# Chlumsky/msdfgen

Hardware: AMD Instinct MI355X
Metric: MSDF glyphs/sec (64x64, fp32) (higher is better)
Workload: dtype f64

## Files before the change

### msdfgen_amd/csrc/msdf_capi.hip

```cpp

#include <hip/hip_runtime.h>

#include <algorithm>
#include <atomic>
#include <chrono>
#include <condition_variable>
#include <cmath>
#include <cstdarg>
#include <cstdio>
#include <cstdlib>
#include <cstring>
#include <deque>
#include <functional>
#include <memory>
#include <mutex>
#include <string>
#include <thread>
#include <vector>

#include <sched.h>

#include "msdf_classplan.hpp"
#include "msdf_hostplan.hpp"
#include "msdf_kernels.hpp"
// ... 645 lines not shown
            rc = fail(MSDFHIP_ERR_HIP, "joining the glyph-class streams failed: %s", hipGetErrorString(joinError));
    }
    if (rc == MSDFHIP_OK && plan.unculled)
        rc = unculled(b, dGlyphs, w, h, dst, toScratch, stream, plan.unculledMapped ? b->work.bucket.ptr+plan.unculledOffset : NULL, plan.unculledCount, call.boxDims);
    return rc;
}

size_t candidateRecords(int nGlyphs, size_t texelsPerGlyph) { return ecHeaderRecords(nGlyphs)+(size_t) nGlyphs*ecSegment(texelsPerGlyph); }
size_t offsetRecords(int nGlyphs) { return (ecOffsetInts(nGlyphs)*sizeof(int)+sizeof(EcCandidate)-1)/sizeof(EcCandidate); }
size_t deferredRecords(int nGlyphs, size_t texelsPerGlyph, int nEdges) {
    return candidateRecords(nGlyphs, texelsPerGlyph)+offsetRecords(nGlyphs)+((size_t) (nEdges > 0 ? nEdges : 1)*2*sizeof(int)+sizeof(EcCandidate)-1)/sizeof(EcCandidate);
}

int ensureDeferred(const MsdfHipBatch *b, size_t cap, EcCandidate **out) {
    std::lock_guard<std::mutex> lock(b->work.mutex);
    HIPCHK(b->work.deferred.ensure(cap));
    HIPCHK(b->work.ecParams.ensure(b->work.glyphCapacity(b->nGlyphs)));
    *out = b->work.deferred.ptr;
    return MSDFHIP_OK;
}

template <int N, bool OVERLAP>
unsigned queryResidentBlocks(int device, size_t lds) {
    enum { LDS_STEP = 2048, LDS_STEPS = 81 };
    static std::atomic<int> cache[LDS_STEPS];
    const size_t step = (lds+LDS_STEP-1)/LDS_STEP;
    return step < LDS_STEPS ? (unsigned) residentBlocks(cache[step], device, reinterpret_cast<const void *>(k_ec_query<N, OVERLAP>), WAVE, step*LDS_STEP) : 0u;
}

template <int N, bool OVERLAP, bool GRES>
int launchEc(const MsdfHipBatch *b, const MsdfHipGlyph *dGlyphs, int w, int h, const float *src, float *out, uint8_t *stencil,
             const MsdfHipConfig &cfg, hipStream_t stream, GenerateCall &call, bool paramsOnly, const EcPlan &p) {
    const int tilesX = (w+TILE-1)/TILE, tiles = tilesOf(w, h);
    const unsigned blocks = (unsigned) b->nGlyphs*(unsigned) tiles;
    if (p.tooManyTexels)
        return fail(MSDFHIP_ERR_INVALID, "batch of %zu texels exceeds the 32-bit texel index of the error-correction pass; split the batch", p.allTexels);
    double *gres = NULL;
    int rc;
    if (GRES) {
        rc = ensureGres(b, (size_t) p.slowGrid*p.resBytes, &gres);
        if (rc != MSDFHIP_OK)
            return rc;
    }
    const size_t gresStride = p.resBytes/sizeof(double);
    const int32_t *dDims = call.boxDims;
    auto slowKernel = k_ec_slow<N, OVERLAP, GRES>;
    auto fastKernel = p.lazyProtect ? k_ec_fast<N, true> : k_ec_fast<N, false>;
    if (call.ecShapeRows) {
        if constexpr (!OVERLAP && !GRES) {
            if (dDims || p.lazyProtect)
                return fail(MSDFHIP_ERR_INVALID, "a correction along the shape's rows takes neither boxes of their own sizes nor the distance check");
            slowKernel = k_ec_slow<N, false, false, true>;
            fastKernel = k_ec_fast<N, false, true>;
        } else
            return fail(MSDFHIP_ERR_INVALID, "a correction along the shape's rows runs without overlap support");
    }
    const auto slowTwin = ecSlowSizedKernel(N, OVERLAP, GRES);
    const auto fastTwin = ecFastSizedKernel(N, p.lazyProtect);
    const auto queryTwin = ecQuerySizedKernel(N, OVERLAP);
    const BatchView v = viewOf(b);
    rc = setLdsTwinned(slowKernel, slowTwin, dDims, p.slowLds);
    if (rc != MSDFHIP_OK)
        return rc;
    ScopedTimer timer(stream, 1, !paramsOnly);
    if (p.route == EC_ROUTE_STAGE_SNAPSHOT || p.route == EC_ROUTE_SLOW_ALL) {
        if (paramsOnly)
            return MSDFHIP_OK;
        launchTwinned(slowKernel, slowTwin, dDims, dim3(p.route == EC_ROUTE_SLOW_ALL ? p.slowGrid : p.snapshotBlocks), p.slowLds, stream, v, dGlyphs, w, h, src, out,
                      stencil, cfg, NULL, 0u, 0, gres, gresStride);
        HIPCHK(hipGetLastError());
        if (p.route == EC_ROUTE_SLOW_ALL)
            countRoute(MSDFHIP_ROUTE_EC_SLOW_ALL);
        return MSDFHIP_OK;
    }
    const unsigned seg = ecSegment((size_t) w*h);
    EcCandidate *deferred = NULL;
    rc = ensureDeferred(b, deferredRecords(b->nGlyphs, (size_t) w*h, b->nEdges), &deferred);
    if (rc != MSDFHIP_OK)
        return rc;
    if (p.route == EC_ROUTE_TOO_COMPLEX)
        return fail(MSDFHIP_ERR_TOO_COMPLEX, "a glyph has %d contours / %d edges: the error-correction pass needs %zu B of LDS per wavefront, device limit is %d B",
                    b->maxContours, b->maxEdges, p.fastLds > p.queryLds ? p.fastLds : p.queryLds, gLdsLimit.load());
    rc = setLdsTwinned(k_ec_query<N, OVERLAP>, queryTwin, dDims, p.queryLds);
    if (rc != MSDFHIP_OK)
        return rc;
    rc = setLdsTwinned(fastKernel, fastTwin, dDims, p.fastLds);
    if (rc != MSDFHIP_OK)
        return rc;
    int *offsets = reinterpret_cast<int *>(deferred+candidateRecords(b->nGlyphs, (size_t) w*h));
    int *corners = reinterpret_cast<int *>(deferred+candidateRecords(b->nGlyphs, (size_t) w*h)+offsetRecords(b->nGlyphs));
    const unsigned queryBlocks = p.residentQueryBlocks(p.staticDeal ? queryResidentBlocks<N, OVERLAP>(b->device, p.queryLds) : 0u);
    const EcQueryPolicy policy = { p.lpcMaxContours, p.lpcEdgeCost, p.lpcMaxEdges, p.lpcMinCount, p.wideMaxEdges, p.wideLoad, p.wideMeanCount, p.gridSteps };
    if (!call.ecParamsQueued)
        hipLaunchKernelGGL(k_ec_params, dim3((unsigned) b->nGlyphs), dim3(WAVE), 0, stream, b->work.ecParams.ptr, viewOf(b), dGlyphs, cfg,
                           reinterpret_cast<unsigned *>(deferred), corners, offsets+ecSizesAt(b->nGlyphs));
    const int *ecOrder = NULL;
    rc = ensureEcOrder(b, &ecOrder, stream);
    if (rc != MSDFHIP_OK)
        return rc;
    if (paramsOnly) {
        HIPCHK(hipGetLastError());
        call.ecParamsQueued = true;
        return MSDFHIP_OK;
    }
    launchTwinned(fastKernel, fastTwin, dDims, dim3(blocks), p.fastLds, stream, v, dGlyphs, w, h, tilesX, tiles, src, out, stencil, cfg, b->work.ecParams.ptr, deferred,
                  seg, b->maxEdges, corners);
    hipLaunchKernelGGL(k_ec_scan, dim3(1), dim3(1024), 0, stream, b->nGlyphs, reinterpret_cast<const unsigned *>(deferred), seg, offsets, policy, ecOrder);
    launchTwinned(k_ec_query<N, OVERLAP>, queryTwin, dDims, dim3(queryBlocks), p.queryLds, stream, v.nGlyphs, v.glyphContourOffsets, v.contourOffsets, v.recs, v.windings,
                  dGlyphs, w, h, src, out, stencil, cfg, b->work.ecParams.ptr, deferred, seg, offsets, offsets+2*(size_t) b->nGlyphs+2, p.queryBatch, p.slotCap,
                  p.slotOffset, policy, call.overflowOut, ecOrder, p.queryFlags);
    if (call.overflowOut)
        call.overflowMirrored = true;
    else
        launchTwinned(slowKernel, slowTwin, dDims, dim3(p.slowGrid), p.slowLds, stream, v, dGlyphs, w, h, src, out, stencil, cfg, deferred, seg, 1, gres, gresStride);
    HIPCHK(hipGetLastError());
    countRoute(ecOrder ? MSDFHIP_ROUTE_EC_QUERY_HEAVIEST : MSDFHIP_ROUTE_EC_QUERY_BATCH);
    if (p.wideSlots)
        countRoute(MSDFHIP_ROUTE_EC_WIDE_SLOTS);
    return MSDFHIP_OK;
}

template <int N>
int dispatchEc(const MsdfHipBatch *b, const MsdfHipGlyph *dGlyphs, int w, int h, const float *src, float *out, uint8_t *stencil,
               const MsdfHipConfig &cfg, hipStream_t stream, GenerateCall &call, bool paramsOnly) {
    const EcPlan p = planCorrection(planEnv(b->device), countsOf(b), w, h, N, cfg.overlap_support != 0, cfg.ec_mode, cfg.ec_distance_check, cfg.ec_stage_limit,
                                    ecFastLdsBytes(b->maxEdges, N));
    if (!cfg.overlap_support)
        return launchEc<N, false, false>(b, dGlyphs, w, h, src, out, stencil, cfg, stream, call, paramsOnly, p);
    return p.gres ? launchEc<N, true, true>(b, dGlyphs, w, h, src, out, stencil, cfg, stream, call, paramsOnly, p)
                  : launchEc<N, true, false>(b, dGlyphs, w, h, src, out, stencil, cfg, stream, call, paramsOnly, p);
}

int checkConfig(const MsdfHipConfig *cfg) {
    if (!cfg)
        return fail(MSDFHIP_ERR_INVALID, "cfg is NULL");
    if (cfg->ec_mode < 0 || cfg->ec_mode > 3 || cfg->ec_distance_check < 0 || cfg->ec_distance_check > 2 || cfg->ec_stage_limit < 0 || cfg->ec_stage_limit > 4)
        return fail(MSDFHIP_ERR_INVALID, "bad error-correction config (mode %d, distance check %d, stage limit %d)", cfg->ec_mode, cfg->ec_distance_check, cfg->ec_stage_limit);
    return MSDFHIP_OK;
}

int ensureScratch(const MsdfHipBatch *b, size_t floats, float **out) {
    std::lock_guard<std::mutex> lock(b->work.mutex);
    HIPCHK(b->work.scratch.ensure(floats));
    *out = b->work.scratch.ptr;
    return MSDFHIP_OK;
}

int runCorrection(const MsdfHipBatch *b, int channels, int w, int h, const MsdfHipGlyph *dGlyphs, const float *src, float *out, uint8_t *stencil,
                  const MsdfHipConfig &cfg, hipStream_t stream, GenerateCall &call, bool paramsOnly) {
    int rc = MSDFHIP_OK;
    forOneOf<3, 4>(channels, [&](auto n) { rc = dispatchEc<decltype(n)::value>(b, dGlyphs, w, h, src, out, stencil, cfg, stream, call, paramsOnly); });
    return rc;
}

int prepareAhead(const MsdfHipBatch *b, int mode, int w, int h, const MsdfHipGlyph *dGlyphs, const MsdfHipConfig *cfg, hipStream_t stream, GenerateCall &call) {
    if (b->nGlyphs == 0 || w == 0 || h == 0)
        return MSDFHIP_OK;
    const int nch = channelsOf(mode);
    int rc = MSDFHIP_OK;
// ... 3105 lines not shown
```

### msdfgen_amd/csrc/msdf_ec_fast.hpp

```cpp
#pragma once

#include "msdf_ec.hpp"

namespace msdfhip {

enum { EC_DEFER = 0x80 };

enum { EC_V_ERROR = 1,
       EC_V_CHECK = 2,
       EC_V_COND = 4,
       EC_V_HELD = 8 };
enum { EC_ORDER_EAGER = 0, EC_ORDER_LAZY = 1, EC_ORDER_LAZY_HELD = 2 };

MSDF_HD bool ecHasBasePass(const EcParams &p) { return p.distanceCheck == EC_DO_NOT_CHECK || (p.distanceCheck == EC_CHECK_AT_EDGE && p.mode != EC_MODE_EDGE_ONLY); }
MSDF_HD bool ecHasShapePass(const EcParams &p) { return p.distanceCheck == EC_ALWAYS_CHECK || p.distanceCheck == EC_CHECK_AT_EDGE; }
MSDF_HD bool ecLazyProtect(const EcParams &p) { return p.mode == EC_MODE_EDGE_PRIORITY && p.distanceCheck == EC_CHECK_AT_EDGE; }

struct FastCtx {
    double span;
    bool p1;
    bool pShape;
    bool basePass, shapePass;
    int order;
};
// ... 138 lines not shown
            break;
        const double t = i ? d.r1 : d.r0;
        const float xm = interpolatedMedianQuad<HWMED>(a, l, q, t);
        int rangeFlags = diagonalUnitFlags<HWMED>(cx, am, dm, a, l, q, t, 0, false, xm);
        if (d.ne > 0)
            rangeFlags |= diagonalUnitFlags<HWMED>(cx, am, dm, a, l, q, t, d.ex0, true, xm);
        if (d.ne > 1)
            rangeFlags |= diagonalUnitFlags<HWMED>(cx, am, dm, a, l, q, t, d.ex1, true, xm);
        if (diagonalRootVerdict(cx, rangeFlags, t, verdict, sink))
            return verdict;
    }
    return verdict;
}

struct Neighbourhood {
    float v[3][3][3];
    float dev[3][3];
    unsigned cls[3][3];
    unsigned valid;
};

template <bool HWMED = false>
MSDF_HD float ecTexelDeviation(const float *t) { return fabsf(medianOf<HWMED>(t[0], t[1], t[2])-.5f); }

enum { EC_CLS_INSIDE = 0x8000 };
MSDF_HD unsigned ecTexelClassWord(const float *t) {
    unsigned w = EC_CLS_INSIDE;
    MSDF_UNROLL
    for (int j = 0; j < 3; ++j) {
        const float d = t[j == 2 ? 0 : j+1]-t[j];
        w |= (d > 0 ? 1u<<j : 0u)|(d < 0 ? 8u<<j : 0u)|(d == 0 ? 64u<<j : 0u);
    }
    return w;
}

MSDF_HD unsigned ecValidFromWords(const Neighbourhood &nb) {
    unsigned valid = 0;
    MSDF_UNROLL
    for (int m = 0; m < 9; ++m)
        valid |= (nb.cls[m/3][m%3]&EC_CLS_INSIDE) ? 1u<<m : 0u;
    return valid;
}

MSDF_HD void loadNeighbourhood(Neighbourhood &nb, const SdfView &sdf, int x, int yn) {
    MSDF_UNROLL
    for (int dy = -1; dy <= 1; ++dy) {
        MSDF_UNROLL
        for (int dx = -1; dx <= 1; ++dx) {
            const int nx = x+dx, ny = yn+dy;
            const bool in = nx >= 0 && ny >= 0 && nx < sdf.w && ny < sdf.h;
            const float *t = sdf.native(in ? nx : x, in ? ny : yn);
            nb.v[dy+1][dx+1][0] = t[0], nb.v[dy+1][dx+1][1] = t[1], nb.v[dy+1][dx+1][2] = t[2];
            nb.dev[dy+1][dx+1] = ecTexelDeviation(t);
            nb.cls[dy+1][dx+1] = in ? ecTexelClassWord(t) : 0u;
        }
    }
    nb.valid = ecValidFromWords(nb);
}

enum { EC_PROTECT_TESTS = 8, EC_PROTECT_MASK = 0x1ef };
MSDF_HD unsigned texelProtectMask(const Neighbourhood &nb, const EcParams &p) {
    const float sdev = nb.dev[1][1];
    unsigned mask = 0;
    MSDF_UNROLL
    for (int dy = -1; dy <= 1; ++dy) {
        MSDF_UNROLL
// ... 235 lines not shown
```

### msdfgen_amd/csrc/msdf_kernels.hpp

```cpp
#pragma once

#include <hip/hip_runtime.h>
#include "msdf_device.hpp"
#include "msdf_prep.hpp"
#include "msdf_ec.hpp"
#include "msdf_ec_fast.hpp"
#include "msdf_cull.hpp"
#include "msdf_scanline.hpp"
#include "msdf_render.hpp"
#include "msdf_qualityplan.hpp"
#include "msdf_shapeprep.hpp"
#include "msdf_frame.hpp"
#include "msdf_legacy.hpp"
#include "../../include/msdfgen_hip.h"

namespace msdfhip {

#ifndef MSDF_DISTANCE_WAVES_PER_SIMD
#define MSDF_DISTANCE_WAVES_PER_SIMD 4
#endif
constexpr int TILE = 8;
constexpr int WAVE = 64;
constexpr int REC_DOUBLES = sizeof(EdgeRec)/sizeof(double);

// ... 974 lines not shown

template <class T, T V>
struct EcConstant {
    static constexpr T value = V;
};

__device__ __forceinline__ int waveInclusiveSum(int v) {
    v += __builtin_amdgcn_update_dpp(0, v, 0x111, 0xf, 0xf, false);
    v += __builtin_amdgcn_update_dpp(0, v, 0x112, 0xf, 0xf, false);
    v += __builtin_amdgcn_update_dpp(0, v, 0x114, 0xf, 0xf, false);
    v += __builtin_amdgcn_update_dpp(0, v, 0x118, 0xf, 0xf, false);
    v += __builtin_amdgcn_update_dpp(0, v, 0x142, 0xa, 0xf, false);
    v += __builtin_amdgcn_update_dpp(0, v, 0x143, 0xc, 0xf, false);
    return v;
}
struct EcWaveReserve {
    int *count;
    __device__ void operator()(int nFirst, int nOthers, int &atFirst, int &atOthers) {
        const int n = nFirst|nOthers<<16;
        const int through = waveInclusiveSum(n);
        const int total = __builtin_amdgcn_readlane(through, WAVE-1), before = through-n;
        *count = (total&0xffff)+(total>>16);
        atFirst = before&0xffff, atOthers = (total&0xffff)+(before>>16);
    }
};
template <unsigned VALID, int TESTS, unsigned FIRST>
__device__ __forceinline__ void ecAppendWave(unsigned short *queue, int *count, unsigned mask, int lane) {
    if (__ballot(mask != 0) == 0)
        return;
    EcWaveReserve reserve = { count };
    ecAppendItems<VALID, TESTS, FIRST>(queue, mask, lane, reserve);
}

template <int N, int ORDER = -1, bool SIZED = false, bool SHAPE_ROWS = false>
__device__ __forceinline__ void ecFastBody(const BatchView &batch, const MsdfHipGlyph *glyphs, int width, int height, int tilesX, int tilesPerGlyph,
          const float *src, float *out, uint8_t *stencilOut, const MsdfHipConfig &cfg, const EcGlyphParams *glyphParams, EcCandidate *cands, unsigned seg,
          int maxEdges, const int *corners, const unsigned blockId, int *smemFast, const int sinkSlots = 0, const int sinkSlot = 0, const int32_t *__restrict__ dims = NULL) {
    const GlyphWork wk = decodeItem(blockId, batch.nGlyphs, tilesPerGlyph);
    if (!wk.valid)
        return;
    const int boxW = SIZED ? MSDF_UNIFORM(dims[2*wk.g]) : width, boxH = SIZED ? MSDF_UNIFORM(dims[2*wk.g+1]) : height;
    if (SIZED && ((wk.tile%tilesX)*TILE >= boxW || (wk.tile/tilesX)*TILE >= boxH))
        return;
    float *halo = reinterpret_cast<float *>(smemFast);
    int *verdictLds = reinterpret_cast<int *>(halo+EC_HALO*EC_HALO*N);
    int *itemCount = verdictLds+WAVE;
    unsigned short *queue = reinterpret_cast<unsigned short *>(itemCount+4);
    unsigned short *protectQueue = queue+EC_QUEUE_CAP;
    struct TexelClass {
        float dev;
        unsigned cls;
    };
    TexelClass *classLds = reinterpret_cast<TexelClass *>(queue+EC_QUEUE_CAP)-EC_HALO*EC_HALO;
    static_assert((EC_QUEUE_CAP*sizeof(unsigned short))%sizeof(TexelClass) == 0 && EC_QUEUE_CAP*sizeof(unsigned short) >= EC_HALO*EC_HALO*sizeof(TexelClass)
                  && 2*WAVE >= EC_HALO*EC_HALO && WAVE%EC_HALO == 4 && WAVE/EC_HALO == 6, "classLds overlays the queue's tail; the halo is staged in two rounds");
    const int lane = threadIdx.x;
    const MsdfHipGlyph gd = glyphs[wk.g];
    EcParams p;
    p.t = loadXform(gd);
    p.minDeviationRatio = cfg.min_deviation_ratio;
    p.minImproveRatio = cfg.min_improve_ratio;
    constexpr bool FOLD = ORDER == 1 && !SIZED;
    p.mode = FOLD ? (int) EC_MODE_EDGE_PRIORITY : cfg.ec_mode, p.distanceCheck = FOLD ? (int) EC_CHECK_AT_EDGE : cfg.ec_distance_check;
    p.overlap = cfg.overlap_support, p.stageLimit = 0;
    const EcGlyphParams gp = glyphParams[wk.g];
    p.hSpan = gp.hSpan, p.vSpan = gp.vSpan, p.dSpan = gp.dSpan, p.texelX = gp.texelX, p.texelY = gp.texelY;
    p.radiusH = gp.radiusH, p.radiusV = gp.radiusV, p.radiusD = gp.radiusD;
    const int tx = wk.tile%tilesX, ty = wk.tile/tilesX;

    const bool lazy = ORDER < 0 ? ecLazyProtect(p) : ORDER != 0;
    bool cornerTexel = false;
    if (p.mode == EC_MODE_EDGE_PRIORITY && !lazy)
        cornerTexel = ecTileCornerTexel(corners+2*(size_t) gp.cornerBegin, gp.nCorners, tx, ty, boxH, gd.flip, lane);

    const ptrdiff_t rowStep = (ptrdiff_t) boxW*N;
    const ptrdiff_t origin = SIZED ? ((ptrdiff_t) wk.g*width*height+(ptrdiff_t) (ty*TILE-1)*boxW+tx*TILE-1)*N : (((ptrdiff_t) wk.g*height+ty*TILE-1)*width+tx*TILE-1)*N;
    const int hr0 = lane/EC_HALO, hc0 = lane-hr0*EC_HALO;
    const ptrdiff_t laneStep0 = hr0*rowStep+hc0*N;
    constexpr bool VOTE = ORDER >= 0 && !SIZED && !SHAPE_ROWS;
    constexpr bool INDEXED = VOTE;
    constexpr float EC_MED3_BOUND = 0x1p100f;
    bool objection = false;
    MSDF_UNROLL
    for (int round = 0; round < 2; ++round) {
        const int idx = lane+round*WAVE;
        const bool wrap = round && hc0+WAVE%EC_HALO >= EC_HALO;
        const int hc = hc0+round*(WAVE%EC_HALO)-(wrap ? EC_HALO : 0), hr = hr0+round*(WAVE/EC_HALO)+(wrap ? 1 : 0);
        const ptrdiff_t laneStep = laneStep0+round*((WAVE/EC_HALO)*rowStep+(WAVE%EC_HALO)*N)+(wrap ? rowStep-EC_HALO*N : 0);
        if (idx < EC_HALO*EC_HALO) {
            const int hx = tx*TILE+hc-1, hy = ty*TILE+hr-1;
            unsigned cls = 0;
            if (hx >= 0 && hy >= 0 && hx < boxW && hy < boxH) {
                const float *t = src+(origin+laneStep);
                float tv[N];
                for (int ch = 0; ch < N; ++ch)
                    tv[ch] = t[ch], halo[idx*N+ch] = tv[ch];
                if (VOTE)
                    objection = objection || !(fabsf(tv[0]) < EC_MED3_BOUND && fabsf(tv[1]) < EC_MED3_BOUND && fabsf(tv[2]) < EC_MED3_BOUND);
                classLds[idx].dev = ecTexelDeviation(tv);
                cls = ecTexelClassWord(tv);
            }
            classLds[idx].cls = cls;
        }
    }
    if (lane < 2)
        itemCount[lane] = 0;
    waveSync();

    const int lx = lane&(TILE-1), ly = lane>>3;
    const int x = tx*TILE+lx, yn = ty*TILE+ly;
    const bool inside = x < boxW && yn < boxH;
    int st = 0;
    const bool classify = inside;
    Neighbourhood nb;
    const int centre = (ly+1)*EC_HALO+lx+1;
    MSDF_UNROLL
    for (int dy = -1; dy <= 1; ++dy) {
        MSDF_UNROLL
        for (int dx = -1; dx <= 1; ++dx) {
            const TexelClass tc = classLds[centre+dy*EC_HALO+dx];
            nb.dev[dy+1][dx+1] = tc.dev, nb.cls[dy+1][dx+1] = tc.cls;
        }
    }
    waveSync();
    unsigned findMask = 0, protectMask = 0;
    const bool hwMedian = VOTE && __ballot(objection) == 0;
    if (classify) {
        MSDF_UNROLL
        for (int dy = -1; dy <= 1; ++dy) {
            MSDF_UNROLL
            for (int dx = -1; dx <= 1; ++dx) {
                const float *t = halo+(centre+dy*EC_HALO+dx)*N;
                nb.v[dy+1][dx+1][0] = t[0], nb.v[dy+1][dx+1][1] = t[1], nb.v[dy+1][dx+1][2] = t[2];
            }
        }
        if (p.mode == EC_MODE_EDGE_PRIORITY && !lazy) {
            if (cornerTexel)
                st |= EC_PROTECTED;
            if (!(st&EC_PROTECTED))
                protectMask = texelProtectMask(nb, p);
        } else if (p.mode == EC_MODE_EDGE_ONLY)
            st |= EC_PROTECTED;
        findMask = hwMedian ? texelCandidateMask<VOTE>(nb) : texelCandidateMask<false>(nb);
    }
    if (p.mode == EC_MODE_EDGE_PRIORITY && !lazy)
        ecAppendWave<EC_PROTECT_MASK, EC_PROTECT_TESTS, EC_PROTECT_MASK>(protectQueue, itemCount+1, protectMask, lane);
    ecAppendWave<EC_FIND_MASK, EC_FIND_TESTS, EC_FIND_LINEAR>(queue, itemCount, findMask, lane);
    verdictLds[lane] = (st&EC_PROTECTED) ? 0x100 : 0;
    waveSync();

    const auto sweep = [&](auto hwmedTag) {
    constexpr bool HWMED = decltype(hwmedTag)::value;
    if (!lazy) {
        ecRunProtectQueue<N, HWMED>(halo, protectQueue, itemCount[1], verdictLds, lane, SHAPE_ROWS && gd.flip);
        waveSync();
    }

    const int nItems = itemCount[0];
    const auto runItems = [&](auto orderTag, const int orderArg) {
        constexpr int CORDER = decltype(orderTag)::value;
        const int order = CORDER >= 0 ? CORDER : orderArg;
        for (int base = 0; base < nItems; base += WAVE) {
            const int it = base+lane;
            if (it >= nItems)
                continue;
            const unsigned item = queue[it];
            const int s = item&63, k = ecItemBit(item)>>2, jp = ecItemBit(item)&3;
            const int word = verdictLds[s];
            if (order == EC_ORDER_LAZY_HELD && (word&(0x100|EC_V_HELD)) != (0x100|EC_V_HELD))
                continue;
            const int sx = s&(TILE-1), sy = s>>3;
            const int dx = ecNeighbourDx(k), dy = ecNeighbourDy(k);
            const float *c = halo+((sy+1)*EC_HALO+sx+1)*N, *n = halo+((sy+1+dy)*EC_HALO+sx+1+dx)*N;
            const float *hb = halo+((sy+1)*EC_HALO+sx+1+dx)*N, *vc = halo+((sy+1+dy)*EC_HALO+sx+1)*N;
            CandidateSink sink;
            sink.header = reinterpret_cast<unsigned *>(cands);
            sink.segment = sinkSlots > 0 ? cands+ecHeaderRecords(sinkSlots)+(size_t) sinkSlot*seg : cands+ecHeaderRecords(batch.nGlyphs)+(size_t) wk.g*seg;
            sink.seg = seg, sink.g = sinkSlots > 0 ? sinkSlot : wk.g;
            sink.texel = (unsigned) (SIZED ? (size_t) wk.g*width*height+(size_t) (ty*TILE+sy)*boxW+tx*TILE+sx : ((size_t) wk.g*height+ty*TILE+sy)*width+tx*TILE+sx);
            const int v = evaluatePair<HWMED, INDEXED, (FOLD || CORDER == EC_ORDER_EAGER) ? CORDER : -1>(c, n, hb, vc, p, (word&0x100) != 0, gd.flip, k, jp, sink, order);
            if (v && order != EC_ORDER_LAZY_HELD)
                atomicOr(&verdictLds[s], v);
        }
    };
    if constexpr (ORDER < 0)
        runItems(EcConstant<int, -1>(), lazy ? EC_ORDER_LAZY : EC_ORDER_EAGER);
    else if constexpr (ORDER == 1)
        runItems(EcConstant<int, EC_ORDER_LAZY>(), EC_ORDER_LAZY);
    else
        runItems(EcConstant<int, EC_ORDER_EAGER>(), EC_ORDER_EAGER);
    waveSync();

    const bool need = lazy && inside && ecNeedsProtection(verdictLds[lane]);
    if (__ballot(need)) {
        __asm__ volatile("" ::: "memory");
        const EcGlyphParams gl = glyphParams[wk.g];
        EcParams pr = p;
        pr.radiusH = gl.radiusH, pr.radiusV = gl.radiusV, pr.radiusD = gl.radiusD;
        cornerTexel = ecTileCornerTexel(corners+2*(size_t) gl.cornerBegin, gl.nCorners, tx, ty, boxH, gd.flip, lane);
        unsigned roundMask = 0;
        if (need) {
            if (cornerTexel)
                verdictLds[lane] |= 0x100;
            else {
                Neighbourhood nd;
                MSDF_UNROLL
                for (int dy = -1; dy <= 1; ++dy) {
                    MSDF_UNROLL
                    for (int dx = -1; dx <= 1; ++dx) {
                        const int nx = x+dx, ny = yn+dy;
// ... 22 lines not shown
                runItems(EcConstant<int, -1>(), EC_ORDER_LAZY_HELD);
            else
                runItems(EcConstant<int, EC_ORDER_LAZY_HELD>(), EC_ORDER_LAZY_HELD);
        }
    }
    };
    if (hwMedian)
        sweep(EcConstant<bool, true>());
    else
        sweep(EcConstant<bool, false>());

    if (!inside)
        return;
    const int verdict = verdictLds[lane];
    if ((verdict&0x100) || (ecHasBasePass(p) && p.distanceCheck == EC_CHECK_AT_EDGE))
        st |= EC_PROTECTED;
    if (verdict&EC_V_ERROR)
        st |= EC_ERROR;
    const size_t texel = SIZED ? (size_t) wk.g*width*height+(size_t) yn*boxW+x : ((size_t) wk.g*height+yn)*width+x;
    const float *in = halo+((ly+1)*EC_HALO+lx+1)*N;
    float v[N];
    for (int i = 0; i < N; ++i)
        v[i] = in[i];
    if (st&EC_ERROR) {
        const float m = medianf(v[0], v[1], v[2]);
        v[0] = m, v[1] = m, v[2] = m;
    }
    float *px = out+gd.out_offset+(ptrdiff_t) gd.row_stride*yn+(ptrdiff_t) N*x;
    for (int i = 0; i < N; ++i)
        px[i] = v[i];
    if (stencilOut)
        stencilOut[stencilIndex(texel, yn, boxW, boxH, cfg.stencil_y_down)] = (uint8_t) st;
}
template <int N, bool LAZY, bool SHAPE_ROWS = false>
__global__ void __launch_bounds__(WAVE, MSDF_EC_FAST_WAVES_PER_SIMD)
k_ec_fast(BatchView batch, const MsdfHipGlyph *glyphs, int width, int height, int tilesX, int tilesPerGlyph,
          const float *src, float *out, uint8_t *stencilOut, MsdfHipConfig cfg, const EcGlyphParams *glyphParams, EcCandidate *cands, unsigned seg,
          int maxEdges, const int *corners) {
    extern __shared__ int smemFast[];
    static_assert(!(LAZY && SHAPE_ROWS), "the lazy order's protection round pairs texels along the bitmap's rows");
    ecFastBody<N, LAZY ? 1 : 0, false, SHAPE_ROWS>(batch, glyphs, width, height, tilesX, tilesPerGlyph, src, out, stencilOut, cfg, glyphParams, cands, seg, maxEdges, corners, blockIdx.x, smemFast);
}

struct EcQueryPolicy { int lpcMaxContours, lpcEdgeCost, lpcMaxEdges, lpcMinCount, wideMaxEdges; float wideLoad, wideMeanCount; int gridSteps; };
MSDF_HD int ecQueryGridSlices(unsigned count, int nE, int C, EcQueryPolicy q) {
    if (q.gridSteps <= 0 || C > q.lpcMaxContours || count == 0)
        return 0;
    int J = 1;
    while (J < (int) count && J < WAVE)
        J <<= 1;
    int S = WAVE/J, need = 1;
    while (need*q.gridSteps < nE && need < WAVE)
        need <<= 1;
    if (need > S)
        S = need;
    return S >= 2 && S <= WAVE/2 ? S : 0;
}
MSDF_HD bool ecQueryLanePerCandidate(unsigned count, int nE, int C, EcQueryPolicy q) {
    if (C > q.lpcMaxContours)
        return false;
    if ((nE > q.lpcMaxEdges && (int) count < q.lpcMinCount))
        return false;
    const long long coop = (long long) count*(340ll*((nE+WAVE-1)/WAVE)+10ll*nE+1000ll);
    const long long lpc = (long long) ((count+WAVE-1)/WAVE)*((long long) q.lpcEdgeCost*nE+1000ll);
    return lpc < coop;
}
MSDF_HD int ecQueryItems(unsigned count, unsigned seg, int nE, int C, EcQueryPolicy lpcMaxContours) {
    if (count > seg)
        return 0;
    const int S = ecQueryGridSlices(count, nE, C, lpcMaxContours);
    if (S)
        return (int) ((count+WAVE/S-1)/(WAVE/S));
    return ecQueryLanePerCandidate(count, nE, C, lpcMaxContours) ? (int) ((count+WAVE-1)/WAVE) : (int) count;
}
// ... 1014 lines not shown
```

### msdfgen_amd/csrc/msdf_launchplan.hpp

```cpp

#pragma once

#include <cstddef>

#include "../../include/msdfgen_hip.h"
#include "msdf_classplan.hpp"

namespace msdfhip {

enum { PLAN_TILE = 8, PLAN_WAVE = 64, PLAN_QUAD = 4, PLAN_DISTANCE_WAVES_PER_SIMD = 4, PLAN_SIMPLE_WAVES_PER_SIMD = 5, PLAN_SIGN_ROWS = PLAN_TILE+2,
       PLAN_PB_SLOT_BYTES = 40 };
const size_t GRES_WORKSPACE_CAP = (size_t) 1<<30;

struct PlanTuning {
    size_t resLdsBudget = (size_t) 10*1024;
    long persistentRounds = 8;
    bool serialClasses = false;
    int querySlotCap = 160, queryLpcContours = 24;
    bool hasQueryLds = false;
    bool hasQueryPolicy = false;
    int qpEdgeCost = 150, qpMaxEdges = 48, qpMinCount = 0x7fffffff, qpWideMaxEdges = 128;
    float qpWideLoad = 4e8f, qpWideMeanCount = 24.f;
    size_t signCap = 192;
    int queryStatic = 2;
// ... 219 lines not shown
    if (nSmall > 0) {
        const bool shortLaunch = env.classTpw() == 1 ||
                                 (size_t) nSmall*(size_t) ((tiles+PLAN_QUAD-1)/PLAN_QUAD) < (size_t) env.t.shortRounds*env.slots(PLAN_DISTANCE_WAVES_PER_SIMD);
        const LdsPlan small = planLds(env, nch, true, classes.smallMaxC, classes.smallMaxE, shortLaunch ? 1 : (int) PLAN_QUAD);
        if (p.refuse(small))
            return p;
        p.add(true, false, shortLaunch ? 1 : (int) PLAN_QUAD, small, shortLaunch ? MSDFHIP_ROUTE_DIST_LDS_SINGLE : MSDFHIP_ROUTE_DIST_LDS_QUAD, nSmall, true, nOne);
    }
    if (nOne > 0) {
        const bool shortLaunch = (size_t) nOne*(size_t) ((tiles+PLAN_QUAD-1)/PLAN_QUAD) < (size_t) env.t.shortRounds*env.slots(PLAN_SIMPLE_WAVES_PER_SIMD);
        const LdsPlan simple = shortLaunch ? shortSimpleLds(env, nch, classes.oneMaxE) : planLds(env, nch, false, 1, classes.oneMaxE);
        if (p.refuse(simple))
            return p;
        p.add(false, shortLaunch, shortLaunch ? 1 : (int) PLAN_QUAD, simple, shortLaunch ? MSDFHIP_ROUTE_DIST_ONE_SINGLE : MSDFHIP_ROUTE_DIST_ONE_QUAD, nOne, true, 0, sOne);
    }
    return p;
}

enum { EC_ROUTE_NORMAL = 0, EC_ROUTE_STAGE_SNAPSHOT, EC_ROUTE_SLOW_ALL, EC_ROUTE_TOO_COMPLEX };
struct EcPlan {
    bool tooManyTexels;
    size_t allTexels;
    bool gres;
    size_t resBytes, slowLds;
    unsigned slowGrid, snapshotBlocks;
    int route;
    int slotCap, mergedCap, slotOffset;
    bool wideSlots;
    int lpcMaxContours, lpcEdgeCost, lpcMaxEdges, lpcMinCount, wideMaxEdges;
    float wideLoad, wideMeanCount;
    int gridSteps;
    size_t queryLds, fastLds;
    bool lazyProtect;
    unsigned queryBlocks;
    bool staticDeal;
    int queryFlags, queryBatch;
    unsigned residentQueryBlocks(unsigned resident) const { return staticDeal && resident && queryBlocks > resident ? resident : queryBlocks; }
};
inline EcPlan planCorrection(const PlanEnv &env, const GlyphCounts &b, int w, int h, int n, bool overlap, int ecMode, int ecCheck, int stageLimit, size_t fastLds) {
    EcPlan p = EcPlan();
    p.allTexels = (size_t) b.nGlyphs*w*h;
    p.tooManyTexels = p.allTexels >= 0xffffffffull;
    p.gres = overlap && (size_t) b.maxContours*PLAN_WAVE*sizeof(double) > 96*1024;
    p.resBytes = overlap ? (size_t) b.maxContours*PLAN_WAVE*sizeof(double) : 0;
    p.slowLds = p.gres ? 0 : p.resBytes;
    p.slowGrid = (unsigned) (p.allTexels/PLAN_WAVE < 64 ? 64 : p.allTexels/PLAN_WAVE > 2048 ? 2048 : p.allTexels/PLAN_WAVE);
    const unsigned cap = p.gres ? p.slowGrid : 16384u;
    p.snapshotBlocks = (unsigned) ((p.allTexels+PLAN_WAVE-1)/PLAN_WAVE < cap ? (p.allTexels+PLAN_WAVE-1)/PLAN_WAVE : cap);
    const int slotCapWanted = env.t.querySlotCap, lpcContoursWanted = env.t.queryLpcContours;
    p.slotCap = b.maxEdges < slotCapWanted ? (b.maxEdges > 0 ? b.maxEdges : 1) : slotCapWanted;
    if (b.nGlyphs < 256 && !env.t.hasQueryLds) {
        const int wide = b.maxEdges < 1024 ? (b.maxEdges > 0 ? b.maxEdges : 1) : 1024;
        const int wideMerged = b.maxContours < wide ? (b.maxContours > 0 ? b.maxContours : 1) : wide;
        if ((size_t) b.maxContours*sizeof(double)+(size_t) (wide+wideMerged)*PLAN_PB_SLOT_BYTES <= (size_t) 64*1024 && wide > p.slotCap)
            p.slotCap = wide, p.wideSlots = true;
    }
    p.lpcMaxContours = b.maxContours < lpcContoursWanted ? b.maxContours : lpcContoursWanted;
    p.lpcEdgeCost = env.t.qpEdgeCost, p.lpcMaxEdges = env.t.qpMaxEdges, p.lpcMinCount = env.t.qpMinCount;
    p.wideMaxEdges = env.t.qpWideMaxEdges, p.wideLoad = env.t.qpWideLoad, p.wideMeanCount = env.t.qpWideMeanCount;
    p.gridSteps = env.t.queryGridSteps;
    const size_t resLanes = overlap ? (size_t) (p.lpcMaxContours > 0 ? p.lpcMaxContours : 1)*PLAN_WAVE*sizeof(double) : 0;
    p.slotOffset = overlap ? (b.maxContours > 0 ? b.maxContours : 1) : 0;
    p.mergedCap = b.maxContours < p.slotCap ? (b.maxContours > 0 ? b.maxContours : 1) : p.slotCap;
    const size_t coopLds = (size_t) p.slotOffset*sizeof(double)+(size_t) (p.slotCap+p.mergedCap)*PLAN_PB_SLOT_BYTES;
    p.queryLds = resLanes > coopLds ? resLanes : coopLds;
    p.fastLds = fastLds;
    if (stageLimit != 0)
        p.route = EC_ROUTE_STAGE_SNAPSHOT;
    else if (p.gres && p.queryLds > env.ldsLimit && fastLds <= env.ldsLimit)
        p.route = EC_ROUTE_SLOW_ALL;
    else if (fastLds > env.ldsLimit || p.queryLds > env.ldsLimit)
        p.route = EC_ROUTE_TOO_COMPLEX;
    p.lazyProtect = ecMode == MSDFHIP_EC_EDGE_PRIORITY && ecCheck == MSDFHIP_CHECK_DISTANCE_AT_EDGE;
    const size_t wanted = p.allTexels/512;
    p.queryBlocks = (unsigned) (wanted < 64 ? 64 : wanted > 8192 ? 8192 : wanted);
    p.staticDeal = env.t.queryStatic != 0;
    p.queryFlags = p.staticDeal ? (env.t.queryStatic == 2 ? 5 : 1) : 0;
    p.queryBatch = env.t.queryBatch;
    return p;
}

struct SignPlan {
    int span, spansX, spans;
    size_t blocks, cap, lds;
    bool wholeRows, chunked;
};
inline SignPlan planSign(const PlanEnv &env, int nGlyphs, int maxEdges, int w, int h) {
    SignPlan p;
    const int tilesX = (w+PLAN_TILE-1)/PLAN_TILE, tilesY = (h+PLAN_TILE-1)/PLAN_TILE;
    p.span = tilesX;
    while (p.span > 1 && (size_t) nGlyphs*tilesY*((tilesX+p.span-1)/p.span) < 4096)
        p.span = (p.span+1)/2;
    p.spansX = (tilesX+p.span-1)/p.span, p.spans = p.spansX*tilesY;
    p.blocks = (size_t) nGlyphs*(size_t) p.spans;
    const size_t capLimit = env.t.signCap;
    const size_t all = 3*(size_t) (maxEdges > 0 ? maxEdges : 1);
    p.cap = all > capLimit ? capLimit : all;
    p.lds = PLAN_SIGN_ROWS*p.cap*(sizeof(double)+sizeof(int))+PLAN_SIGN_ROWS*sizeof(int);
    p.wholeRows = p.span == tilesX, p.chunked = p.cap < all;
    return p;
}

struct LegacyDistancePlan {
    size_t blocks;
    bool tooManyBlocks;
};
// ... 23 lines not shown
```

Baseline: 2.048 million.

## Process four error-correction tiles per wavefront in the fast sweep

The fast error-correction kernel can now loop over four tiles of the same glyph per wavefront. Per-glyph parameters (transform, spans, corner ranges) are loaded once per wave and reused across the four tiles, and halo loads use 32-bit byte offsets with a bounds-check-free path for interior tiles. Median deviation evaluation is deferred until the hardware-median ballot is known. The launch uses fewer blocks, which may reduce parallelism and latency hiding for small batches; the planner keeps one tile per wave below a small-launch threshold.

```diff
diff --git a/msdfgen_amd/csrc/msdf_capi.hip b/msdfgen_amd/csrc/msdf_capi.hip
--- a/msdfgen_amd/csrc/msdf_capi.hip
+++ b/msdfgen_amd/csrc/msdf_capi.hip
@@ -701,7 +701,6 @@
 int launchEc(const MsdfHipBatch *b, const MsdfHipGlyph *dGlyphs, int w, int h, const float *src, float *out, uint8_t *stencil,
              const MsdfHipConfig &cfg, hipStream_t stream, GenerateCall &call, bool paramsOnly, const EcPlan &p) {
     const int tilesX = (w+TILE-1)/TILE, tiles = tilesOf(w, h);
-    const unsigned blocks = (unsigned) b->nGlyphs*(unsigned) tiles;
     if (p.tooManyTexels)
         return fail(MSDFHIP_ERR_INVALID, "batch of %zu texels exceeds the 32-bit texel index of the error-correction pass; split the batch", p.allTexels);
     double *gres = NULL;
@@ -724,6 +723,11 @@
         } else
             return fail(MSDFHIP_ERR_INVALID, "a correction along the shape's rows runs without overlap support");
     }
+    if (p.fastTpw != 1) {
+        if (p.fastTpw != (int) QUAD || dDims || call.ecShapeRows)
+            return fail(MSDFHIP_ERR_INVALID, "the correction sweep has no form of %d tiles per wavefront for this call", p.fastTpw);
+        fastKernel = p.lazyProtect ? k_ec_fast<N, true, false, (int) QUAD> : k_ec_fast<N, false, false, (int) QUAD>;
+    }
     const auto slowTwin = ecSlowSizedKernel(N, OVERLAP, GRES);
     const auto fastTwin = ecFastSizedKernel(N, p.lazyProtect);
     const auto queryTwin = ecQuerySizedKernel(N, OVERLAP);
@@ -772,7 +776,7 @@
         call.ecParamsQueued = true;
         return MSDFHIP_OK;
     }
-    launchTwinned(fastKernel, fastTwin, dDims, dim3(blocks), p.fastLds, stream, v, dGlyphs, w, h, tilesX, tiles, src, out, stencil, cfg, b->work.ecParams.ptr, deferred,
+    launchTwinned(fastKernel, fastTwin, dDims, dim3((unsigned) p.fastBlocks), p.fastLds, stream, v, dGlyphs, w, h, tilesX, tiles, src, out, stencil, cfg, b->work.ecParams.ptr, deferred,
                   seg, b->maxEdges, corners);
     hipLaunchKernelGGL(k_ec_scan, dim3(1), dim3(1024), 0, stream, b->nGlyphs, reinterpret_cast<const unsigned *>(deferred), seg, offsets, policy, ecOrder);
     launchTwinned(k_ec_query<N, OVERLAP>, queryTwin, dDims, dim3(queryBlocks), p.queryLds, stream, v.nGlyphs, v.glyphContourOffsets, v.contourOffsets, v.recs, v.windings,
@@ -793,7 +797,7 @@
 int dispatchEc(const MsdfHipBatch *b, const MsdfHipGlyph *dGlyphs, int w, int h, const float *src, float *out, uint8_t *stencil,
                const MsdfHipConfig &cfg, hipStream_t stream, GenerateCall &call, bool paramsOnly) {
     const EcPlan p = planCorrection(planEnv(b->device), countsOf(b), w, h, N, cfg.overlap_support != 0, cfg.ec_mode, cfg.ec_distance_check, cfg.ec_stage_limit,
-                                    ecFastLdsBytes(b->maxEdges, N));
+                                    ecFastLdsBytes(b->maxEdges, N), !call.boxDims && !call.ecShapeRows);
     if (!cfg.overlap_support)
         return launchEc<N, false, false>(b, dGlyphs, w, h, src, out, stencil, cfg, stream, call, paramsOnly, p);
     return p.gres ? launchEc<N, true, true>(b, dGlyphs, w, h, src, out, stencil, cfg, stream, call, paramsOnly, p)
diff --git a/msdfgen_amd/csrc/msdf_ec_fast.hpp b/msdfgen_amd/csrc/msdf_ec_fast.hpp
--- a/msdfgen_amd/csrc/msdf_ec_fast.hpp
+++ b/msdfgen_amd/csrc/msdf_ec_fast.hpp
@@ -194,6 +194,10 @@
         w |= (d > 0 ? 1u<<j : 0u)|(d < 0 ? 8u<<j : 0u)|(d == 0 ? 64u<<j : 0u);
     }
     return w;
+}
+
+MSDF_HD bool ecHaloInside(int tx, int ty, int tile, int boxW, int boxH) {
+    return tx > 0 && ty > 0 && tx*tile+tile < boxW && ty*tile+tile < boxH;
 }
 
 MSDF_HD unsigned ecValidFromWords(const Neighbourhood &nb) {
diff --git a/msdfgen_amd/csrc/msdf_kernels.hpp b/msdfgen_amd/csrc/msdf_kernels.hpp
--- a/msdfgen_amd/csrc/msdf_kernels.hpp
+++ b/msdfgen_amd/csrc/msdf_kernels.hpp
@@ -1030,15 +1030,41 @@
     ecAppendItems<VALID, TESTS, FIRST>(queue, mask, lane, reserve);
 }
 
-template <int N, int ORDER = -1, bool SIZED = false, bool SHAPE_ROWS = false>
-__device__ __forceinline__ void ecFastBody(const BatchView &batch, const MsdfHipGlyph *glyphs, int width, int height, int tilesX, int tilesPerGlyph,
+struct EcFastWave {
+    int g, boxW, boxH;
+    MsdfHipGlyph gd;
+    EcParams p;
+    int cornerBegin, nCorners;
+    bool lazy;
+};
+template <int N, int ORDER, bool SIZED>
+__device__ __forceinline__ EcFastWave ecFastWave(const MsdfHipGlyph *glyphs, const int g, int width, int height, const MsdfHipConfig &cfg,
+                                                 const EcGlyphParams *glyphParams, const int32_t *__restrict__ dims) {
+    EcFastWave w;
+    w.g = g;
+    w.boxW = SIZED ? MSDF_UNIFORM(dims[2*g]) : width, w.boxH = SIZED ? MSDF_UNIFORM(dims[2*g+1]) : height;
+    w.gd = glyphs[g];
+    w.p.t = loadXform(w.gd);
+    w.p.minDeviationRatio = cfg.min_deviation_ratio;
+    w.p.minImproveRatio = cfg.min_improve_ratio;
+    constexpr bool FOLD = ORDER == 1 && !SIZED;
+    w.p.mode = FOLD ? (int) EC_MODE_EDGE_PRIORITY : cfg.ec_mode, w.p.distanceCheck = FOLD ? (int) EC_CHECK_AT_EDGE : cfg.ec_distance_check;
+    w.p.overlap = cfg.overlap_support, w.p.stageLimit = 0;
+    const EcGlyphParams gp = glyphParams[g];
+    w.p.hSpan = gp.hSpan, w.p.vSpan = gp.vSpan, w.p.dSpan = gp.dSpan, w.p.texelX = gp.texelX, w.p.texelY = gp.texelY;
+    w.p.radiusH = gp.radiusH, w.p.radiusV = gp.radiusV, w.p.radiusD = gp.radiusD;
+    w.cornerBegin = gp.cornerBegin, w.nCorners = gp.nCorners;
+    w.lazy = ORDER < 0 ? ecLazyProtect(w.p) : ORDER != 0;
+    return w;
+}
+
+template <int N, int ORDER, bool SIZED, bool SHAPE_ROWS, bool LOOPED>
+__device__ __forceinline__ void ecFastTile(const EcFastWave &wave, const int tx, const int ty, const int nGlyphs, int width, int height, int tilesX,
           const float *src, float *out, uint8_t *stencilOut, const MsdfHipConfig &cfg, const EcGlyphParams *glyphParams, EcCandidate *cands, unsigned seg,
-          int maxEdges, const int *corners, const unsigned blockId, int *smemFast, const int sinkSlots = 0, const int sinkSlot = 0, const int32_t *__restrict__ dims = NULL) {
-    const GlyphWork wk = decodeItem(blockId, batch.nGlyphs, tilesPerGlyph);
-    if (!wk.valid)
-        return;
-    const int boxW = SIZED ? MSDF_UNIFORM(dims[2*wk.g]) : width, boxH = SIZED ? MSDF_UNIFORM(dims[2*wk.g+1]) : height;
-    if (SIZED && ((wk.tile%tilesX)*TILE >= boxW || (wk.tile/tilesX)*TILE >= boxH))
+          const int *corners, int *smemFast, const int sinkSlots, const int sinkSlot) {
+    struct { int g; } wk = { wave.g };
+    const int boxW = wave.boxW, boxH = wave.boxH;
+    if (SIZED && (tx*TILE >= boxW || ty*TILE >= boxH))
         return;
     float *halo = reinterpret_cast<float *>(smemFast);
     int *verdictLds = reinterpret_cast<int *>(halo+EC_HALO*EC_HALO*N);
@@ -1052,24 +1078,16 @@
     TexelClass *classLds = reinterpret_cast<TexelClass *>(queue+EC_QUEUE_CAP)-EC_HALO*EC_HALO;
     static_assert((EC_QUEUE_CAP*sizeof(unsigned short))%sizeof(TexelClass) == 0 && EC_QUEUE_CAP*sizeof(unsigned short) >= EC_HALO*EC_HALO*sizeof(TexelClass)
                   && 2*WAVE >= EC_HALO*EC_HALO && WAVE%EC_HALO == 4 && WAVE/EC_HALO == 6, "classLds overlays the queue's tail; the halo is staged in two rounds");
-    const int lane = threadIdx.x;
-    const MsdfHipGlyph gd = glyphs[wk.g];
-    EcParams p;
-    p.t = loadXform(gd);
-    p.minDeviationRatio = cfg.min_deviation_ratio;
-    p.minImproveRatio = cfg.min_improve_ratio;
+    int lane = threadIdx.x;
+    if (LOOPED)
+        __asm__ volatile("" : "+v"(lane));
+    const MsdfHipGlyph &gd = wave.gd;
+    const EcParams &p = wave.p;
     constexpr bool FOLD = ORDER == 1 && !SIZED;
-    p.mode = FOLD ? (int) EC_MODE_EDGE_PRIORITY : cfg.ec_mode, p.distanceCheck = FOLD ? (int) EC_CHECK_AT_EDGE : cfg.ec_distance_check;
-    p.overlap = cfg.overlap_support, p.stageLimit = 0;
-    const EcGlyphParams gp = glyphParams[wk.g];
-    p.hSpan = gp.hSpan, p.vSpan = gp.vSpan, p.dSpan = gp.dSpan, p.texelX = gp.texelX, p.texelY = gp.texelY;
-    p.radiusH = gp.radiusH, p.radiusV = gp.radiusV, p.radiusD = gp.radiusD;
-    const int tx = wk.tile%tilesX, ty = wk.tile/tilesX;
-
-    const bool lazy = ORDER < 0 ? ecLazyProtect(p) : ORDER != 0;
+    const bool lazy = wave.lazy;
     bool cornerTexel = false;
     if (p.mode == EC_MODE_EDGE_PRIORITY && !lazy)
-        cornerTexel = ecTileCornerTexel(corners+2*(size_t) gp.cornerBegin, gp.nCorners, tx, ty, boxH, gd.flip, lane);
+        cornerTexel = ecTileCornerTexel(corners+2*(size_t) wave.cornerBegin, wave.nCorners, tx, ty, boxH, gd.flip, lane);
 
     const ptrdiff_t rowStep = (ptrdiff_t) boxW*N;
     const ptrdiff_t origin = SIZED ? ((ptrdiff_t) wk.g*width*height+(ptrdiff_t) (ty*TILE-1)*boxW+tx*TILE-1)*N : (((ptrdiff_t) wk.g*height+ty*TILE-1)*width+tx*TILE-1)*N;
@@ -1079,26 +1097,52 @@
     constexpr bool INDEXED = VOTE;
     constexpr float EC_MED3_BOUND = 0x1p100f;
     bool objection = false;
+    const char *originBytes = reinterpret_cast<const char *>(src+origin);
+    const unsigned rowBytes = (unsigned) boxW*(unsigned) (N*sizeof(float)), laneBytes0 = (unsigned) hr0*rowBytes+(unsigned) hc0*(unsigned) (N*sizeof(float));
+    constexpr bool DEFER = LOOPED && VOTE;
+    float kept[2][3];
+    bool staged[2] = { false, false };
+    const auto stage = [&](auto interiorTag) {
+    constexpr bool INTERIOR = decltype(interiorTag)::value;
     MSDF_UNROLL
     for (int round = 0; round < 2; ++round) {
         const int idx = lane+round*WAVE;
         const bool wrap = round && hc0+WAVE%EC_HALO >= EC_HALO;
         const int hc = hc0+round*(WAVE%EC_HALO)-(wrap ? EC_HALO : 0), hr = hr0+round*(WAVE/EC_HALO)+(wrap ? 1 : 0);
         const ptrdiff_t laneStep = laneStep0+round*((WAVE/EC_HALO)*rowStep+(WAVE%EC_HALO)*N)+(wrap ? rowStep-EC_HALO*N : 0);
+        const unsigned laneBytes = laneBytes0+round*((WAVE/EC_HALO)*rowBytes+(WAVE%EC_HALO)*N*(unsigned) sizeof(float))
+                                   +(wrap ? rowBytes-EC_HALO*N*(unsigned) sizeof(float) : 0u);
         if (idx < EC_HALO*EC_HALO) {
             const int hx = tx*TILE+hc-1, hy = ty*TILE+hr-1;
             unsigned cls = 0;
-            if (hx >= 0 && hy >= 0 && hx < boxW && hy < boxH) {
-                const float *t = src+(origin+laneStep);
+            if (INTERIOR || (hx >= 0 && hy >= 0 && hx < boxW && hy < boxH)) {
+                const float *t = LOOPED ? reinterpret_cast<const float *>(originBytes+laneBytes) : src+(origin+laneStep);
                 float tv[N];
                 for (int ch = 0; ch < N; ++ch)
                     tv[ch] = t[ch], halo[idx*N+ch] = tv[ch];
                 if (VOTE)
                     objection = objection || !(fabsf(tv[0]) < EC_MED3_BOUND && fabsf(tv[1]) < EC_MED3_BOUND && fabsf(tv[2]) < EC_MED3_BOUND);
-                classLds[idx].dev = ecTexelDeviation(tv);
+                if (DEFER)
+                    kept[round][0] = tv[0], kept[round][1] = tv[1], kept[round][2] = tv[2], staged[round] = true;
+                else
+                    classLds[idx].dev = ecTexelDeviation(tv);
                 cls = ecTexelClassWord(tv);
             }
             classLds[idx].cls = cls;
+        }
+    }
+    };
+    if (LOOPED && ecHaloInside(tx, ty, TILE, boxW, boxH))
+        stage(EcConstant<bool, true>());
+    else
+        stage(EcConstant<bool, false>());
+    const bool hwMedian = VOTE && __ballot(objection) == 0;
+    if (DEFER) {
+        MSDF_UNROLL
+        for (int round = 0; round < 2; ++round) {
+            const int idx = lane+round*WAVE;
+            if (staged[round])
+                classLds[idx].dev = hwMedian ? ecTexelDeviation<true>(kept[round]) : ecTexelDeviation<false>(kept[round]);
         }
     }
     if (lane < 2)
@@ -1122,7 +1166,6 @@
     }
     waveSync();
     unsigned findMask = 0, protectMask = 0;
-    const bool hwMedian = VOTE && __ballot(objection) == 0;
     if (classify) {
         MSDF_UNROLL
         for (int dy = -1; dy <= 1; ++dy) {
@@ -1173,7 +1216,7 @@
             const float *hb = halo+((sy+1)*EC_HALO+sx+1+dx)*N, *vc = halo+((sy+1+dy)*EC_HALO+sx+1)*N;
             CandidateSink sink;
             sink.header = reinterpret_cast<unsigned *>(cands);
-            sink.segment = sinkSlots > 0 ? cands+ecHeaderRecords(sinkSlots)+(size_t) sinkSlot*seg : cands+ecHeaderRecords(batch.nGlyphs)+(size_t) wk.g*seg;
+            sink.segment = sinkSlots > 0 ? cands+ecHeaderRecords(sinkSlots)+(size_t) sinkSlot*seg : cands+ecHeaderRecords(nGlyphs)+(size_t) wk.g*seg;
             sink.seg = seg, sink.g = sinkSlots > 0 ? sinkSlot : wk.g;
             sink.texel = (unsigned) (SIZED ? (size_t) wk.g*width*height+(size_t) (ty*TILE+sy)*boxW+tx*TILE+sx : ((size_t) wk.g*height+ty*TILE+sy)*width+tx*TILE+sx);
             const int v = evaluatePair<HWMED, INDEXED, (FOLD || CORDER == EC_ORDER_EAGER) ? CORDER : -1>(c, n, hb, vc, p, (word&0x100) != 0, gd.flip, k, jp, sink, order);
@@ -1262,14 +1305,42 @@
     if (stencilOut)
         stencilOut[stencilIndex(texel, yn, boxW, boxH, cfg.stencil_y_down)] = (uint8_t) st;
 }
-template <int N, bool LAZY, bool SHAPE_ROWS = false>
+template <int N, int ORDER = -1, bool SIZED = false, bool SHAPE_ROWS = false>
+__device__ __forceinline__ void ecFastBody(const BatchView &batch, const MsdfHipGlyph *glyphs, int width, int height, int tilesX, int tilesPerGlyph,
+          const float *src, float *out, uint8_t *stencilOut, const MsdfHipConfig &cfg, const EcGlyphParams *glyphParams, EcCandidate *cands, unsigned seg,
+          int maxEdges, const int *corners, const unsigned blockId, int *smemFast, const int sinkSlots = 0, const int sinkSlot = 0, const int32_t *__restrict__ dims = NULL) {
+    const GlyphWork wk = decodeItem(blockId, batch.nGlyphs, tilesPerGlyph);
+    if (!wk.valid)
+        return;
+    const EcFastWave wave = ecFastWave<N, ORDER, SIZED>(glyphs, wk.g, width, height, cfg, glyphParams, dims);
+    ecFastTile<N, ORDER, SIZED, SHAPE_ROWS, false>(wave, wk.tile%tilesX, wk.tile/tilesX, batch.nGlyphs, width, height, tilesX, src, out, stencilOut, cfg, glyphParams, cands, seg, corners, smemFast,
+                                                   sinkSlots, sinkSlot);
+}
+template <int N, bool LAZY, bool SHAPE_ROWS = false, int TPW = 1>
 __global__ void __launch_bounds__(WAVE, MSDF_EC_FAST_WAVES_PER_SIMD)
 k_ec_fast(BatchView batch, const MsdfHipGlyph *glyphs, int width, int height, int tilesX, int tilesPerGlyph,
           const float *src, float *out, uint8_t *stencilOut, MsdfHipConfig cfg, const EcGlyphParams *glyphParams, EcCandidate *cands, unsigned seg,
           int maxEdges, const int *corners) {
     extern __shared__ int smemFast[];
     static_assert(!(LAZY && SHAPE_ROWS), "the lazy order's protection round pairs texels along the bitmap's rows");
-    ecFastBody<N, LAZY ? 1 : 0, false, SHAPE_ROWS>(batch, glyphs, width, height, tilesX, tilesPerGlyph, src, out, stencilOut, cfg, glyphParams, cands, seg, maxEdges, corners, blockIdx.x, smemFast);
+    static_assert(TPW == 1 || (TPW == (int) QUAD && !SHAPE_ROWS), "one tile per wavefront, or four");
+    if constexpr (TPW == 1)
+        ecFastBody<N, LAZY ? 1 : 0, false, SHAPE_ROWS>(batch, glyphs, width, height, tilesX, tilesPerGlyph, src, out, stencilOut, cfg, glyphParams, cands, seg, maxEdges, corners, blockIdx.x, smemFast);
+    else {
+        const GlyphWork wk = decodeItem(blockIdx.x, batch.nGlyphs, (tilesPerGlyph+TPW-1)/TPW);
+        if (!wk.valid)
+            return;
+        const EcFastWave wave = ecFastWave<N, LAZY ? 1 : 0, false>(glyphs, wk.g, width, height, cfg, glyphParams, NULL);
+        const int first = wk.tile*TPW, last = first+TPW < tilesPerGlyph ? first+TPW : tilesPerGlyph;
+        int tx = first%tilesX, ty = first/tilesX;
+        MSDF_NOUNROLL
+        for (int tile = first; tile < last; ++tile) {
+            ecFastTile<N, LAZY ? 1 : 0, false, false, true>(wave, tx, ty, batch.nGlyphs, width, height, tilesX, src, out, stencilOut, cfg, glyphParams, cands, seg, corners, smemFast, 0, 0);
+            waveSync();
+            if (++tx == tilesX)
+                tx = 0, ++ty;
+        }
+    }
 }
 
 struct EcQueryPolicy { int lpcMaxContours, lpcEdgeCost, lpcMaxEdges, lpcMinCount, wideMaxEdges; float wideLoad, wideMeanCount; int gridSteps; };
diff --git a/msdfgen_amd/csrc/msdf_launchplan.hpp b/msdfgen_amd/csrc/msdf_launchplan.hpp
--- a/msdfgen_amd/csrc/msdf_launchplan.hpp
+++ b/msdfgen_amd/csrc/msdf_launchplan.hpp
@@ -275,12 +275,15 @@
     int gridSteps;
     size_t queryLds, fastLds;
     bool lazyProtect;
+    int fastTpw;
+    size_t fastBlocks;
     unsigned queryBlocks;
     bool staticDeal;
     int queryFlags, queryBatch;
     unsigned residentQueryBlocks(unsigned resident) const { return staticDeal && resident && queryBlocks > resident ? resident : queryBlocks; }
 };
-inline EcPlan planCorrection(const PlanEnv &env, const GlyphCounts &b, int w, int h, int n, bool overlap, int ecMode, int ecCheck, int stageLimit, size_t fastLds) {
+inline EcPlan planCorrection(const PlanEnv &env, const GlyphCounts &b, int w, int h, int n, bool overlap, int ecMode, int ecCheck, int stageLimit, size_t fastLds,
+                             bool quadForm = true) {
     EcPlan p = EcPlan();
     p.allTexels = (size_t) b.nGlyphs*w*h;
     p.tooManyTexels = p.allTexels >= 0xffffffffull;
@@ -315,6 +318,10 @@
     else if (fastLds > env.ldsLimit || p.queryLds > env.ldsLimit)
         p.route = EC_ROUTE_TOO_COMPLEX;
     p.lazyProtect = ecMode == MSDFHIP_EC_EDGE_PRIORITY && ecCheck == MSDFHIP_CHECK_DISTANCE_AT_EDGE;
+    const size_t tilesAll = (size_t) b.nGlyphs*(size_t) tilesOf(w, h);
+    const bool narrowSpan = (size_t) (PLAN_TILE+2)*(size_t) w*(size_t) n*sizeof(float) < ((size_t) 1<<32);
+    p.fastTpw = quadForm && narrowSpan && tilesAll > (size_t) env.t.smallLaunchTiles ? (int) PLAN_QUAD : 1;
+    p.fastBlocks = distanceBlocks(b.nGlyphs, w, h, p.fastTpw);
     const size_t wanted = p.allTexels/512;
     p.queryBlocks = (unsigned) (wanted < 64 ? 64 : wanted > 8192 ? 8192 : wanted);
     p.staticDeal = env.t.queryStatic != 0;
```

Measured after the change: 2.059 million, median of 6. About the same (+0.5%).
